# stevebottos/owl-vit-object-detection

Hardware: AMD Instinct MI355X
Metric: train images/sec, OWL-ViT-B/16 768x768 (higher is better)
Workload: dtype bf16; 1 GPU; owlvit-base-patch16 bf16, batch=32/GPU, 768x768, full train step (matcher+loss+backward+AdamW); global_batch=32, parallelism=dp1, encoder_streams=2, weights=init, optimizer_schedule=in-line, windows=1

## Files before the change

### owl-vit-object-detection_amd/csrc/gemm_common.h

```cpp
#pragma once
#include "common.h"

constexpr int NUM_CUS = 256;

enum {
    EPI_BIAS_BF16 = 0,
    EPI_QGELU_BF16 = 1,
    EPI_GELU_BF16 = 2,
    EPI_RESID_F32 = 3,
    EPI_F32 = 4,
    EPI_ATOMIC_F32 = 5,
    EPI_TRANS_BF16 = 6,
    EPI_PATCH_F32 = 7,
    EPI_DQGELU_BF16 = 8,
    EPI_DGELU_BF16 = 9,
    EPI_ACC_F32 = 10,
    EPI_SLAB_F32 = 11,
    EPI_PATCHM_F32 = 12,
};

struct GemmP {
    const bf16_t* A; int64_t lda; int64_t a_rows;
    const bf16_t* W; int64_t ldw; int64_t w_rows;
    const float* bias;
// ... 121 lines not shown
        *(float4*)((float*)p.out + orow * p.ldo + n) = make_float4(r4.x + v[0], r4.y + v[1], r4.z + v[2], r4.w + v[3]);
    } else if constexpr (EPI == EPI_F32) {
        *(float4*)((float*)p.out + orow * p.ldo + n) = make_float4(v[0], v[1], v[2], v[3]);
    } else if constexpr (EPI == EPI_SLAB_F32) {
        *(float4*)((float*)p.out + (int64_t)split * p.slab_stride + orow * p.ldo + n) = make_float4(v[0], v[1], v[2], v[3]);
    } else if constexpr (EPI == EPI_PATCH_F32 || EPI == EPI_PATCHM_F32) {
        const float4 p4 = *(const float4*)(posrow + n);
        *(float4*)((float*)p.out + orow * p.ldo + n) = make_float4(v[0] + p4.x, v[1] + p4.y, v[2] + p4.z, v[3] + p4.w);
    } else if constexpr (EPI == EPI_ATOMIC_F32) {
        float* o = (float*)p.out + orow * p.ldo + n;
#pragma unroll
        for (int e = 0; e < 4; e++) atomicAdd(o + e, v[e]);
    }
}

template <int EPI>
__device__ __forceinline__ void epi_pass(const GemmP& p, const f32x16& t0, const f32x16& t1, unsigned char* pieceA,
                                         unsigned char* pieceB, int64_t row_base, int64_t col_base, int lane, int split) {
    constexpr bool TRANS = (EPI == EPI_TRANS_BF16);
    const int hi = lane >> 5, r = lane & 31;
    unsigned char* wrow = (r < 16 ? pieceA : pieceB) + (r & 15) * 256;
#pragma unroll
    for (int qd = 0; qd < 4; qd++) {
        const int c0 = 2 * qd + hi, c1 = 8 + c0;
        *(float4*)(wrow + ((c0 ^ (r & 15)) << 4)) = make_float4(t0[qd * 4 + 0], t0[qd * 4 + 1], t0[qd * 4 + 2], t0[qd * 4 + 3]);
        *(float4*)(wrow + ((c1 ^ (r & 15)) << 4)) = make_float4(t1[qd * 4 + 0], t1[qd * 4 + 1], t1[qd * 4 + 2], t1[qd * 4 + 3]);
    }
    const int ch = lane & 15;
#pragma unroll
    for (int it = 0; it < 8; it++) {
        const int row = it * 4 + (lane >> 4);
        const unsigned char* rrow = (row < 16 ? pieceA : pieceB) + (row & 15) * 256;
        const f32x4 f = lds_read_f4(rrow + ((ch ^ (row & 15)) << 4));
        float v[4] = {f[0], f[1], f[2], f[3]};
        if constexpr (!TRANS) {
            const int64_t m = row_base + row, n = col_base + ch * 4;
            if (m >= p.M || n >= p.N) continue;
            int64_t orow = m;
            const float* posrow = nullptr;
            if constexpr (EPI == EPI_PATCH_F32 || EPI == EPI_PATCHM_F32) {
                const int64_t b = m / p.P, pp = m - b * p.P;
                orow = b * p.Tp + 1 + pp;
                posrow = p.pos + (1 + pp) * p.N;
            }
            epi_quad<EPI>(p, orow, posrow, n, v, split);
        } else {
            const int64_t n = row_base + row, m = col_base + ch * 4;
            if (n >= p.N || m >= p.M) continue;
            const float bv = p.bias ? p.bias[n] : 0.f;
            const int64_t b = m / p.Tp, t = m - b * p.Tp;
            uint2 o;
            o.x = pack_bf2(v[0] + bv, v[1] + bv);
            o.y = pack_bf2(v[2] + bv, v[3] + bv);
            *(uint2*)((bf16_t*)p.out + (b * p.N + n) * p.Tp + t) = o;
        }
    }
}

__device__ __forceinline__ void epi_bias_preload(const float* lds_bias, int hi, f32x4 (&bq)[2][4]) {
    const unsigned a = (unsigned)(uintptr_t)LPTR(lds_bias + 4 * hi);
    asm volatile("ds_read_b128 %0, %8\n\tds_read_b128 %1, %8 offset:32\n\tds_read_b128 %2, %8 offset:64\n\tds_read_b128 %3, %8 offset:96\n\t"
                 "ds_read_b128 %4, %8 offset:128\n\tds_read_b128 %5, %8 offset:160\n\tds_read_b128 %6, %8 offset:192\n\tds_read_b128 %7, %8 offset:224\n\t"
                 "s_waitcnt lgkmcnt(0)"
                 : "=&v"(bq[0][0]), "=&v"(bq[0][1]), "=&v"(bq[0][2]), "=&v"(bq[0][3]), "=&v"(bq[1][0]), "=&v"(bq[1][1]), "=&v"(bq[1][2]), "=&v"(bq[1][3])
                 : "v"(a) : "memory");
}

template <bool GUARD>
__device__ __forceinline__ void epi_aux_load(const GemmP& p, int64_t m_tile, int64_t n_tile, int lane, uint4 (&a)[2]) {
    const int hi = lane >> 5;
    const int64_t m = m_tile + (lane & 31);
#pragma unroll
    for (int c = 0; c < 2; c++) {
        const int64_t n = n_tile + 16 * c + 8 * hi;
        a[c] = make_uint4(0u, 0u, 0u, 0u);
        if (!GUARD || (m < p.M && n < p.N)) a[c] = *(const uint4*)((const bf16_t*)p.aux + m * p.ld_aux + n);
    }
}

template <int EPI, bool GUARD>
__device__ __forceinline__ void epi_tile_bf16(const GemmP& p, const f32x16& acc, int64_t m_tile, int64_t n_tile, int lane,
                                              uint4& chunk0, uint4& chunk1, const float* lds_bias, const uint4* aux_pre = nullptr,
                                              const f32x4* bias_pre = nullptr) {
    constexpr bool TRANS = (EPI == EPI_TRANS_BF16);
    const int hi = lane >> 5;
    unsigned w[8];
    unsigned aw[8] = {};
    if constexpr (TRANS) {
        const int64_t n = n_tile + (lane & 31);
        float bv = 0.f;
        if (p.bias) bv = lds_read_f1(lds_bias + (lane & 31));
#pragma unroll
        for (int qd = 0; qd < 4; qd++) {
            w[2 * qd] = pack_bf2(acc[qd * 4 + 0] + bv, acc[qd * 4 + 1] + bv);
            w[2 * qd + 1] = pack_bf2(acc[qd * 4 + 2] + bv, acc[qd * 4 + 3] + bv);
        }
    } else {
        const int64_t m = m_tile + (lane & 31);
        const bool m_ok = !GUARD || m < p.M;
        const bf16_t* aux_row = (const bf16_t*)p.aux + m * p.ld_aux + n_tile + 4 * hi;
        const float* bias_p = lds_bias + 4 * hi;
        if constexpr (EPI == EPI_DQGELU_BF16 || EPI == EPI_DGELU_BF16) {
            if (aux_pre) {
                unsigned ax[4] = {aux_pre[0].x, aux_pre[0].y, aux_pre[1].x, aux_pre[1].y}, ay[4] = {aux_pre[0].z, aux_pre[0].w, aux_pre[1].z, aux_pre[1].w};
#pragma unroll
                for (int k = 0; k < 4; k++) {
                    auto r = __builtin_amdgcn_permlane32_swap(ax[k], ay[k], false, false);
                    ax[k] = r[0]; ay[k] = r[1];
                }
                aw[0] = ax[0]; aw[1] = ax[1]; aw[2] = ay[0]; aw[3] = ay[1]; aw[4] = ax[2]; aw[5] = ax[3]; aw[6] = ay[2]; aw[7] = ay[3];
            }
        }
#pragma unroll
        for (int qd = 0; qd < 4; qd++) {
            float v[4];
            const bool n_ok = !GUARD || (n_tile + 8 * qd + 4 * hi) < p.N;
            const bool ok = m_ok && n_ok;
            const f32x2_t al = {p.alpha, p.alpha};
            f32x2_t b01 = {0.f, 0.f}, b23 = {0.f, 0.f};
            if (p.bias) {
                const f32x4 b4 = bias_pre ? bias_pre[qd] : lds_read_f4(bias_p + 8 * qd);
                b01 = (f32x2_t){b4[0], b4[1]}; b23 = (f32x2_t){b4[2], b4[3]};
            }
            const f32x2_t v01 = __builtin_elementwise_fma((f32x2_t){acc[qd * 4 + 0], acc[qd * 4 + 1]}, al, b01);
            const f32x2_t v23 = __builtin_elementwise_fma((f32x2_t){acc[qd * 4 + 2], acc[qd * 4 + 3]}, al, b23);
            v[0] = v01.x; v[1] = v01.y; v[2] = v23.x; v[3] = v23.y;
            if constexpr (EPI == EPI_QGELU_BF16 || EPI == EPI_GELU_BF16) {
                float sv[4] = {v[0], v[1], v[2], v[3]};
                if constexpr (EPI == EPI_QGELU_BF16) {
#pragma unroll
                    for (int e = 0; e < 4; e += 2) {
                        const f32x2_t u = {v[e], v[e + 1]};
                        const f32x2_t t = u * -2.4554669595930156f;
                        const f32x2_t d = (f32x2_t){__builtin_amdgcn_exp2f(t.x), __builtin_amdgcn_exp2f(t.y)} + 1.0f;
                        const f32x2_t r = {__builtin_amdgcn_rcpf(d.x), __builtin_amdgcn_rcpf(d.y)};
                        const f32x2_t o = u * r;
                        if (p.aux) { sv[e] = dqgelu_from_s(u.x, r.x); sv[e + 1] = dqgelu_from_s(u.y, r.y); }
                        v[e] = o.x; v[e + 1] = o.y;
                    }
                } else {
#pragma unroll
                    for (int e = 0; e < 4; e++) v[e] = gelu_f(v[e]);
                }
                if (p.aux) {
                    if constexpr (EPI == EPI_QGELU_BF16) {
                        aw[2 * qd] = pack_bf2(sv[0], sv[1]); aw[2 * qd + 1] = pack_bf2(sv[2], sv[3]);
                    } else {
                        uint2 a; a.x = pack_bf2(sv[0], sv[1]); a.y = pack_bf2(sv[2], sv[3]);
                        if (ok) *(uint2*)((bf16_t*)aux_row + 8 * qd) = a;
                    }
                }
            } else if constexpr (EPI == EPI_DQGELU_BF16 || EPI == EPI_DGELU_BF16) {
                uint2 a = make_uint2(0u, 0u);
                if (aux_pre) a = make_uint2(aw[2 * qd], aw[2 * qd + 1]);
                else if (ok) a = *(const uint2*)(aux_row + 8 * qd);
                const float u[4] = {bf2f(a.x & 0xffff), bf2f(a.x >> 16), bf2f(a.y & 0xffff), bf2f(a.y >> 16)};
#pragma unroll
                for (int e = 0; e < 4; e++) v[e] *= (EPI == EPI_DQGELU_BF16) ? u[e] : dgelu_f(u[e]);
            }
            w[2 * qd] = pack_bf2(v[0], v[1]);
            w[2 * qd + 1] = pack_bf2(v[2], v[3]);
        }
    }
    if constexpr (!TRANS && EPI == EPI_QGELU_BF16) {
        if (p.aux) {
            unsigned ax[4] = {aw[0], aw[1], aw[4], aw[5]}, ay[4] = {aw[2], aw[3], aw[6], aw[7]};
#pragma unroll
            for (int k = 0; k < 4; k++) {
                auto r = __builtin_amdgcn_permlane32_swap(ax[k], ay[k], false, false);
                ax[k] = r[0]; ay[k] = r[1];
            }
            typedef __attribute__((ext_vector_type(4))) unsigned u32x4_t;
            const int64_t m = m_tile + (lane & 31);
            bf16_t* arow = (bf16_t*)p.aux + m * p.ld_aux + n_tile + 8 * hi;
            const u32x4_t s0 = {ax[0], ax[1], ay[0], ay[1]}, s1 = {ax[2], ax[3], ay[2], ay[3]};
            if (!GUARD || (m < p.M && n_tile + 8 * hi < p.N)) *(u32x4_t*)arow = s0;
            if (!GUARD || (m < p.M && n_tile + 16 + 8 * hi < p.N)) *(u32x4_t*)(arow + 16) = s1;
        }
    }
    unsigned x[4] = {w[0], w[1], w[4], w[5]}, y[4] = {w[2], w[3], w[6], w[7]};
#pragma unroll
    for (int k = 0; k < 4; k++) {
        auto r = __builtin_amdgcn_permlane32_swap(x[k], y[k], false, false);
        x[k] = r[0]; y[k] = r[1];
    }
    chunk0 = make_uint4(x[0], x[1], y[0], y[1]);
    chunk1 = make_uint4(x[2], x[3], y[2], y[3]);
}


__device__ __forceinline__ void epi_lines_bias_preload(const float* lds_bias, int hi, f32x4 (&bq)[8]) {
    const unsigned a = (unsigned)(uintptr_t)LPTR(lds_bias + 32 * hi);
    asm volatile("ds_read_b128 %0, %8\n\tds_read_b128 %1, %8 offset:16\n\tds_read_b128 %2, %8 offset:32\n\tds_read_b128 %3, %8 offset:48\n\t"
                 "ds_read_b128 %4, %8 offset:64\n\tds_read_b128 %5, %8 offset:80\n\tds_read_b128 %6, %8 offset:96\n\tds_read_b128 %7, %8 offset:112\n\t"
                 "s_waitcnt lgkmcnt(0)"
                 : "=&v"(bq[0]), "=&v"(bq[1]), "=&v"(bq[2]), "=&v"(bq[3]), "=&v"(bq[4]), "=&v"(bq[5]), "=&v"(bq[6]), "=&v"(bq[7])
                 : "v"(a) : "memory");
}

__device__ __forceinline__ void quad_transpose16(unsigned (&d)[16], int lane) {
    const bool o1 = lane & 1, o2 = lane & 2;
#pragma unroll
    for (int c = 0; c < 4; c++) {
#pragma unroll
        for (int g = 0; g < 2; g++) {
            unsigned& x = d[8 * g + c]; unsigned& y = d[8 * g + 4 + c];
            const unsigned u = (unsigned)__builtin_amdgcn_mov_dpp((int)(o1 ? x : y), 0xB1, 0xF, 0xF, true);
            if (o1) x = u; else y = u;
        }
#pragma unroll
        for (int g = 0; g < 2; g++) {
            unsigned& x = d[4 * g + c]; unsigned& y = d[4 * g + 8 + c];
            const unsigned u = (unsigned)__builtin_amdgcn_mov_dpp((int)(o2 ? x : y), 0x4E, 0xF, 0xF, true);
            if (o2) x = u; else y = u;
        }
    }
}

template <bool GUARD>
__device__ __forceinline__ void epi_lines_aux_load(const GemmP& p, int64_t m_tile, int64_t n_wave, int lane, unsigned (&x)[16]) {
    typedef __attribute__((ext_vector_type(4))) unsigned u32x4_t;
    const int hi = lane >> 5;
    const bf16_t* base = (const bf16_t*)p.aux + m_tile * p.ld_aux + n_wave;
    const unsigned ld = (unsigned)p.ld_aux, col = 32u * hi + 8u * (lane & 3), r0 = (unsigned)(lane & 28);
#pragma unroll
    for (int t = 0; t < 4; t++) {
        u32x4_t v = {0u, 0u, 0u, 0u};
        if (!GUARD || (m_tile + r0 + t < p.M && n_wave + col < p.N)) v = *(const u32x4_t*)(base + ((r0 + t) * ld + col));
        x[4 * t] = v[0]; x[4 * t + 1] = v[1]; x[4 * t + 2] = v[2]; x[4 * t + 3] = v[3];
    }
}

template <int EPI, bool GUARD>
__device__ __forceinline__ void epi_lines_bf16(const GemmP& p, const f32x16& acc0, const f32x16& acc1, int64_t m_tile, int64_t n_wave, int lane,
                                               const float* lds_bias, const f32x4* bias_pre = nullptr,
                                               unsigned* aux_words = nullptr) {
    static_assert(EPI == EPI_BIAS_BF16 || EPI == EPI_QGELU_BF16 || EPI == EPI_GELU_BF16 || EPI == EPI_DQGELU_BF16,
                  "quad-contiguous epilogue: forward bf16 epilogues and the multiply-by-saved-derivative one");
    const int hi = lane >> 5;
    const int64_t m = m_tile + (lane & 31);
    const float* bias_p = lds_bias + 32 * hi;
    unsigned d_own[16], a[16];
    unsigned (&d)[16] = (EPI == EPI_DQGELU_BF16) ? *reinterpret_cast<unsigned (*)[16]>(aux_words) : d_own;
#pragma unroll
    for (int j = 0; j < 2; j++)
#pragma unroll
        for (int qd = 0; qd < 4; qd++) {
            const f32x16& acc = j ? acc1 : acc0;
            float v[4];
            const f32x2_t al = {p.alpha, p.alpha};
            f32x2_t b01 = {0.f, 0.f}, b23 = {0.f, 0.f};
            if (p.bias) {
                const f32x4 b4 = bias_pre ? bias_pre[4 * j + qd] : lds_read_f4(bias_p + 16 * j + 4 * qd);
                b01 = (f32x2_t){b4[0], b4[1]}; b23 = (f32x2_t){b4[2], b4[3]};
            }
            const f32x2_t v01 = __builtin_elementwise_fma((f32x2_t){acc[qd * 4 + 0], acc[qd * 4 + 1]}, al, b01);
            const f32x2_t v23 = __builtin_elementwise_fma((f32x2_t){acc[qd * 4 + 2], acc[qd * 4 + 3]}, al, b23);
            v[0] = v01.x; v[1] = v01.y; v[2] = v23.x; v[3] = v23.y;
            if constexpr (EPI == EPI_QGELU_BF16 || EPI == EPI_GELU_BF16) {
                float sv[4] = {v[0], v[1], v[2], v[3]};
                if constexpr (EPI == EPI_QGELU_BF16) {
#pragma unroll
                    for (int e = 0; e < 4; e += 2) {
                        const f32x2_t u = {v[e], v[e + 1]};
                        const f32x2_t t = u * -2.4554669595930156f;
                        const f32x2_t dd = (f32x2_t){__builtin_amdgcn_exp2f(t.x), __builtin_amdgcn_exp2f(t.y)} + 1.0f;
                        const f32x2_t r = {__builtin_amdgcn_rcpf(dd.x), __builtin_amdgcn_rcpf(dd.y)};
                        const f32x2_t o = u * r;
                        if (p.aux) { sv[e] = dqgelu_from_s(u.x, r.x); sv[e + 1] = dqgelu_from_s(u.y, r.y); }
                        v[e] = o.x; v[e + 1] = o.y;
                    }
                } else {
#pragma unroll
                    for (int e = 0; e < 4; e++) v[e] = gelu_f(v[e]);
                }
                if (p.aux) { a[8 * j + 2 * qd] = pack_bf2(sv[0], sv[1]); a[8 * j + 2 * qd + 1] = pack_bf2(sv[2], sv[3]); }
            } else if constexpr (EPI == EPI_DQGELU_BF16) {
                const unsigned a0 = aux_words[8 * j + 2 * qd], a1 = aux_words[8 * j + 2 * qd + 1];
                v[0] *= bf2f(a0 & 0xffff); v[1] *= bf2f(a0 >> 16); v[2] *= bf2f(a1 & 0xffff); v[3] *= bf2f(a1 >> 16);
            }
            d[8 * j + 2 * qd] = pack_bf2(v[0], v[1]);
            d[8 * j + 2 * qd + 1] = pack_bf2(v[2], v[3]);
        }
    typedef __attribute__((ext_vector_type(4))) unsigned u32x4_t;
    if constexpr (EPI == EPI_QGELU_BF16 || EPI == EPI_GELU_BF16) {
        if (p.aux) {
            bf16_t* aux_row = (bf16_t*)p.aux + m * p.ld_aux + n_wave + 32 * hi;
#pragma unroll
            for (int t = 0; t < 4; t++)
                if (!GUARD || (m < p.M && n_wave + 32 * hi + 8 * t < p.N))
                    *(u32x4_t*)(aux_row + 8 * t) = (u32x4_t){a[4 * t], a[4 * t + 1], a[4 * t + 2], a[4 * t + 3]};
        }
    }
    quad_transpose16(d, lane);
    const int64_t row0 = m_tile + (lane & 28), n = n_wave + 32 * hi + 8 * (lane & 3);
#pragma unroll
    for (int t = 0; t < 4; t++) {
        const int64_t row = row0 + t;
        if (GUARD && (row >= p.M || n >= p.N)) continue;
        *(u32x4_t*)((bf16_t*)p.out + row * p.ldo + n) = (u32x4_t){d[4 * t], d[4 * t + 1], d[4 * t + 2], d[4 * t + 3]};
    }
}

template <int EPI, bool GUARD>
__device__ __forceinline__ void epi_tile_f32(const GemmP& p, const f32x16& acc, int64_t m_tile, int64_t n_tile, int lane, const float* lds_bias,
                                             const f32x4* bias_pre = nullptr) {
    const int hi = lane >> 5;
    const int64_t m = m_tile + (lane & 31);
    const bool m_ok = !GUARD || m < p.M;
    float* orow = (float*)p.out + m * p.ldo + n_tile + 4 * hi;
    const float* bias_p = lds_bias + 4 * hi;
#pragma unroll
    for (int qd = 0; qd < 4; qd++) {
        float v[4];
#pragma unroll
        for (int e = 0; e < 4; e++) v[e] = acc[qd * 4 + e] * p.alpha;
        if (p.bias) {
            const f32x4 b4 = bias_pre ? bias_pre[qd] : lds_read_f4(bias_p + 8 * qd);
            v[0] += b4[0]; v[1] += b4[1]; v[2] += b4[2]; v[3] += b4[3];
        }
        const bool ok = m_ok && (!GUARD || (n_tile + 8 * qd + 4 * hi) < p.N);
        if (!ok) continue;
        if constexpr (EPI == EPI_ACC_F32) {
            const float4 r4 = *(const float4*)(orow + 8 * qd);
            *(float4*)(orow + 8 * qd) = make_float4(r4.x + v[0], r4.y + v[1], r4.z + v[2], r4.w + v[3]);
        } else {
            *(float4*)(orow + 8 * qd) = make_float4(v[0], v[1], v[2], v[3]);
        }
    }
}

template <bool GUARD>
__device__ __forceinline__ void epi_tile_patch(const GemmP& p, const f32x16& acc, int64_t m_tile, int64_t n_tile, int lane) {
    const int hi = lane >> 5;
    const int64_t m = m_tile + (lane & 31);
    const bool m_ok = !GUARD || m < p.M;
    const int64_t mm = m_ok ? m : 0;
    const int64_t b = mm / p.P, pp = mm - b * p.P;
    float* orow = (float*)p.out + (b * p.Tp + 1 + pp) * p.ldo + n_tile + 4 * hi;
    const float* prow = p.pos + (1 + pp) * p.N + n_tile + 4 * hi;
#pragma unroll
    for (int qd = 0; qd < 4; qd++) {
        if (!m_ok || (GUARD && (n_tile + 8 * qd + 4 * hi) >= p.N)) continue;
        const float4 p4 = *(const float4*)(prow + 8 * qd);
        *(float4*)(orow + 8 * qd) = make_float4(acc[qd * 4 + 0] * p.alpha + p4.x, acc[qd * 4 + 1] * p.alpha + p4.y,
                                                acc[qd * 4 + 2] * p.alpha + p4.z, acc[qd * 4 + 3] * p.alpha + p4.w);
    }
}

template <int EPI, bool GUARD>
__device__ __forceinline__ void epi_store_chunk(const GemmP& p, const uint4& ch, int64_t m_tile, int64_t n_tile, int c, int lane) {
    const int hi = lane >> 5;
    if constexpr (EPI == EPI_TRANS_BF16) {
        const int64_t n = n_tile + (lane & 31), m = m_tile + 16 * c + 8 * hi;
        if (GUARD && (n >= p.N || m >= p.M)) return;
        const int64_t b = m / p.Tp, t = m - b * p.Tp;
        *(uint4*)((bf16_t*)p.out + (b * p.N + n) * p.Tp + t) = ch;
    } else {
        int64_t m = m_tile + (lane & 31), n = n_tile + 16 * c + 8 * hi;
        if (GUARD && (m >= p.M || n >= p.N)) return;
#ifdef OWL_TUNING
        if (p.dbg & 2) { m = (int64_t)(blockIdx.x & 255) * 256 + (m & 255); n &= 255; }
#endif
        typedef __attribute__((ext_vector_type(4))) unsigned u32x4_t;
        u32x4_t* dst = (u32x4_t*)((bf16_t*)p.out + m * p.ldo + n);
        const u32x4_t val = {ch.x, ch.y, ch.z, ch.w};
#ifdef OWL_TUNING
        if (p.dbg & 4) { __builtin_nontemporal_store(val, dst); return; }
#endif
        *dst = val;
    }
}
```

### owl-vit-object-detection_amd/csrc/gemm_pp2.hip

```cpp
#include "gemm_common.h"
#include <type_traits>

static constexpr int QBM = 256, QBN = 256, QBK = 64;
static constexpr int Q_A_BYTES = QBM * QBK * 2, Q_B_BYTES = QBN * QBK * 2, Q_STAGE = Q_A_BYTES + Q_B_BYTES;
static constexpr int Q_BIAS_OFF = 2 * Q_STAGE, Q_LDS = 2 * Q_STAGE + 2 * 1024;

template <int N> __device__ __forceinline__ void q_wait() { asm volatile("s_waitcnt vmcnt(%0) lgkmcnt(0)" ::"n"(N) : "memory"); }
__device__ __forceinline__ void q_wait_lgkm() { asm volatile("s_waitcnt lgkmcnt(0)" ::: "memory"); }
__device__ __forceinline__ void q_bar() {
    __builtin_amdgcn_sched_barrier(0);
    __builtin_amdgcn_s_barrier();
    asm volatile("" ::: "memory");
    __builtin_amdgcn_sched_barrier(0);
}

template <int EPI, bool TRACE = false, bool LINES = false>
__global__ __launch_bounds__(512) void gemm_pp2_kernel(GemmP p) {
    extern __shared__ __attribute__((aligned(16))) unsigned char lds[];
    const int lane = threadIdx.x & 63;
    const int w = __builtin_amdgcn_readfirstlane(threadIdx.x >> 6);
    const int hi = lane >> 5;
    const int grp = w >> 2, wc = w & 3;
    const int nk = (int)(p.K / QBK);
    const int nitems = p.tiles_m * p.tiles_n;
    const int bw = p.nsplit;
    auto decode = [&](int it, int& tm, int& tn) {
        const int per_block = p.tiles_m * bw;
        const int cb = it / per_block, rem = it - cb * per_block;
        tm = rem / bw; tn = cb * bw + (rem - tm * bw);
    };
    int item, item_end, item_step;
    if (p.persistent) {
        const int xcd = blockIdx.x & 7, idx = blockIdx.x >> 3, chunk = (nitems + 7) >> 3;
        item = xcd * chunk + idx; item_end = min(nitems, (xcd + 1) * chunk); item_step = gridDim.x >> 3;
    } else {
        item = xcd_remap(blockIdx.x, nitems); item_end = item + 1; item_step = 1;
    }
    if (item >= item_end) return;
    if (p.stagger > 0 && ((blockIdx.x >> 3) & 1))
        for (int i = 0; i < p.stagger; i++) __builtin_amdgcn_s_sleep(127);
#ifdef OWL_TUNING
    const bool abl_nodma = (p.dbg >> 16) & 1, abl_noread = (p.dbg >> 17) & 1, abl_noepi = (p.dbg >> 18) & 1;
    bool abl_prologue = true;
#else
    constexpr bool abl_nodma = false, abl_noread = false, abl_noepi = false, abl_prologue = true;
#endif

    int a_item = item, a_k = 0, a_buf = 0;
    int b_item = item, b_k = 0, b_buf = 0, b_parity = 0;
    unsigned a_voff[2][2], w_voff[2][2], b_voff = 0;
    const bf16_t* a_base = nullptr;
    const bf16_t* w_base = nullptr;
    const float* b_base = nullptr;
    const bool has_bias = p.bias != nullptr;
    constexpr bool GATHER = (EPI == EPI_PATCH_F32);
    const bool np2 = GATHER && p.ps != (int64_t(1) << p.ps_log2);
    int a_j[2] = {0, 0};
    auto stage_A = [&]() {
        if (a_k == 0) {
            int tm, tn_unused; decode(a_item, tm, tn_unused);
            const int64_t m0 = (int64_t)tm * QBM;
            a_base = GATHER ? p.A : p.A + m0 * p.lda;
#pragma unroll
            for (int h = 0; h < 2; h++)
#pragma unroll
                for (int q = 0; q < 2; q++) {
                    const int r = h * 128 + (w * 2 + q) * 8 + (lane >> 3);
                    const int c = (lane & 7) ^ ((r >> 1) & 7);
                    int64_t am = m0 + r; if (am >= p.a_rows) am = p.a_rows - 1;
                    if constexpr (GATHER) {
                        const unsigned P32 = (unsigned)p.P, G32 = (unsigned)p.G, S32 = (unsigned)p.S, ps32 = (unsigned)p.ps;
                        const unsigned b = (unsigned)am / P32, pp = (unsigned)am - b * P32;
                        const unsigned py = pp / G32, px = pp - py * G32;
                        unsigned ky = (unsigned)(c * 8) >> p.ps_log2, kx = (unsigned)(c * 8) & ((1u << p.ps_log2) - 1u);
                        if (np2) { a_j[q] = (int)ky; ky = 0; kx = min(kx, ps32 - 8u); }
                        a_voff[h][q] = ((((b * 3u) * S32 + py * ps32 + ky) * S32) + px * ps32 + kx) * 2u;
                    } else {
                        a_voff[h][q] = (unsigned)(((am - m0) * p.lda + c * 8) * 2);
                    }
                }
        }
        unsigned char* base = lds + a_buf * Q_STAGE;
        int64_t koff = (int64_t)a_k * QBK;
        unsigned roff[2] = {0u, 0u};
        if constexpr (GATHER) {
            if (np2) {
                koff = 0;
#pragma unroll
                for (int q = 0; q < 2; q++) {
                    unsigned R = (unsigned)(a_k * (QBK >> p.ps_log2) + a_j[q]);
                    R = min(R, 3u * (unsigned)p.ps - 1u);
                    const unsigned ch = (R * (unsigned)p.ps_magic) >> 16, ky = R - ch * (unsigned)p.ps;
                    roff[q] = ((ch * (unsigned)p.S + ky) * (unsigned)p.S) * 2u;
                }
            } else {
                const int k = a_k * QBK;
                const int ch = k >> (2 * p.ps_log2), ky = (k & ((1 << (2 * p.ps_log2)) - 1)) >> p.ps_log2;
                koff = ((int64_t)ch * p.S + ky) * p.S;
            }
        }
        const unsigned char* g = (const unsigned char*)(a_base + koff);
        if (!abl_nodma || abl_prologue) {
#pragma unroll
        for (int h = 0; h < 2; h++)
#pragma unroll
            for (int q = 0; q < 2; q++)
                __builtin_amdgcn_global_load_lds(GPTR(g + (a_voff[h][q] + roff[q])), LPTR(base + (h * 128 + (w * 2 + q) * 8) * 128), 16, 0, 0);
        }
        a_buf ^= 1;
        if (++a_k == nk) { a_k = 0; a_item += item_step; }
    };
    auto stage_B = [&]() -> int {
        const bool first = b_k == 0;
        if (first) {
            int tm, tn; decode(b_item, tm, tn);
            const int64_t n0 = (int64_t)tn * QBN;
            w_base = p.W + n0 * p.ldw;
#pragma unroll
            for (int h = 0; h < 2; h++)
#pragma unroll
                for (int q = 0; q < 2; q++) {
                    const int r = h * 128 + (w * 2 + q) * 8 + (lane >> 3);
                    const int c = (lane & 7) ^ ((r >> 1) & 7);
                    const int rs = LINES ? ((r & ~63) | (((r >> 2) & 1) << 5) | (((r >> 5) & 1) << 4) | (((r >> 3) & 3) << 2) | (r & 3)) : r;
                    int64_t wn = n0 + rs; if (wn >= p.w_rows) wn = p.w_rows - 1;
                    w_voff[h][q] = (unsigned)(((wn - n0) * p.ldw + c * 8) * 2);
                }
            if (has_bias) {
                int64_t n = n0 + lane * 4; if (n + 4 > p.N) n = p.N - 4;
                b_base = p.bias + n0;
                b_voff = (unsigned)((n - n0) * 4);
            }
        }
        unsigned char* base = lds + b_buf * Q_STAGE + Q_A_BYTES;
        const unsigned char* g = (const unsigned char*)(w_base + (int64_t)b_k * QBK);
        int n_ops = 0;
        if (!abl_nodma || abl_prologue) {
#pragma unroll
        for (int h = 0; h < 2; h++)
#pragma unroll
            for (int q = 0; q < 2; q++)
                __builtin_amdgcn_global_load_lds(GPTR(g + w_voff[h][q]), LPTR(base + (h * 128 + (w * 2 + q) * 8) * 128), 16, 0, 0);
        n_ops = 4;
        if (first && has_bias) {
            __builtin_amdgcn_global_load_lds(GPTR((const unsigned char*)b_base + b_voff), LPTR(lds + Q_BIAS_OFF + b_parity * 1024), 16, 0, 0);
            n_ops = 5;
        }
        }
        b_buf ^= 1;
        if (++b_k == nk) { b_k = 0; b_item += item_step; b_parity ^= 1; }
        return n_ops;
    };

    const int a_frag_off = frag_off<false>(grp * 128, lane), b_frag_off = Q_A_BYTES + frag_off<true>(wc * 64, lane);

    stage_B(); stage_A(); stage_B();
    q_wait<4>();
    q_bar();
#ifdef OWL_TUNING
    abl_prologue = false;
#endif

    int cur = 0, tile_parity = 0;
    const bool tr_wg = TRACE && blockIdx.x == 0;
    bool tr_first = false;
    int tr_tile = 0;
    if (TRACE && (p.dbg >> 8) == 0) tr_first = true;
    unsigned long long tr_ts[12] = {};
    bool a_early = false;
    int pending_stores = 0;
    constexpr bool STAGGERED_EPI = ((EPI == EPI_BIAS_BF16 && !LINES) || EPI == EPI_F32 || EPI == EPI_ACC_F32 || EPI == EPI_PATCH_F32 || EPI == EPI_PATCHM_F32);
    if (STAGGERED_EPI && grp == 1) q_bar();
    unsigned long long wg_t0 = 0;
    unsigned long long wg_r0 = 0;
    if constexpr (TRACE) asm volatile("s_memtime %0\n\ts_memrealtime %1\n\ts_waitcnt lgkmcnt(0)" : "=s"(wg_t0), "=s"(wg_r0) :: "memory");
    unsigned long long tile_ts[5] = {};
    auto tile_stamp = [&](int i) {
        if constexpr (TRACE) { if (tr_wg && tr_first) asm volatile("s_memtime %0\n\ts_waitcnt lgkmcnt(0)" : "=s"(tile_ts[i]) :: "memory"); }
    };
    while (true) {
        tile_stamp(0);
        AccBlock blk[4][2];
#pragma unroll
        for (int i = 0; i < 4; i++)
#pragma unroll
            for (int j = 0; j < 2; j++) acc_block_zero(blk[i][j]);
        int tm, tn; decode(item, tm, tn);
        const int64_t cm0 = (int64_t)tm * QBM, cn0 = (int64_t)tn * QBN;
        if (!STAGGERED_EPI && grp == 1) q_bar();
        tile_stamp(1);
        for (int kt = 0; kt < nk; kt++) {
            const unsigned char* tb = lds + cur * Q_STAGE;
            auto stamp = [&](int idx) {
                if constexpr (TRACE) {
                    if (tr_wg && tr_first && kt == ((p.dbg >> 4) & 15)) {
                        if (idx == 1 || idx == 6) return;
                        if (idx == 0 || idx == 2 || idx == 7 || idx >= 10) asm volatile("s_memtime %0\n\ts_waitcnt lgkmcnt(0)" : "=s"(tr_ts[idx]));
                        else asm volatile("s_memtime %0" : "=s"(tr_ts[idx]));
                    }
                }
            };
            bf16x8 fa[2][4], fb[2][4];
            auto ld_a = [&](int ih) {
#pragma unroll
                for (int t = 0; t < 2; t++)
#pragma unroll
                    for (int x = 0; x < 4; x++) fa[t][x] = frag_read(tb + (2 * ih + t) * 4096, a_frag_off, x >> 1, x & 1);
            };
            auto mma = [&](int ih) {
                __builtin_amdgcn_s_setprio(1);
#pragma unroll
                for (int s = 0; s < 2; s++)
#pragma unroll
                    for (int t = 0; t < 2; t++)
#pragma unroll
                        for (int j = 0; j < 2; j++) mma_block_step(blk[2 * ih + t][j], fb[j], fa[t], s);
                __builtin_amdgcn_s_setprio(0);
            };
            stamp(0);
            if (!abl_noread || kt == 0) {
#pragma unroll
            for (int j = 0; j < 2; j++)
#pragma unroll
                for (int x = 0; x < 4; x++) fb[j][x] = frag_read(tb + j * 4096, b_frag_off, x >> 1, x & 1);
            ld_a(0);
            }
            if (a_early) a_early = false;
            else if (a_item < item_end) stage_A();
            stamp(1);
            q_wait_lgkm();
            stamp(2);
            q_bar();
            stamp(3);
            mma(0);
            stamp(4);
            q_bar();
            stamp(5);
            if (!abl_noread || kt == 0) ld_a(1);
            int n_new = 0;
            if (b_item < item_end) n_new = stage_B();
            stamp(6);
            switch (n_new + pending_stores) {
                case 4: q_wait<4>(); break;
                case 5: q_wait<5>(); break;
                case 20: q_wait<20>(); break;
                case 21: q_wait<21>(); break;
                case 36: q_wait<36>(); break;
                case 37: q_wait<37>(); break;
                default: q_wait<0>(); break;
            }
            pending_stores = 0;
            stamp(7);
            q_bar();
            stamp(8);
            mma(1);
            stamp(9);
            q_bar();
            stamp(10);
            if constexpr (TRACE) {
                if (tr_wg && tr_first && kt == ((p.dbg >> 4) & 15) && lane == 0) {
#pragma unroll
                    for (int i = 0; i < 11; i++) ((unsigned long long*)(lds + Q_LDS))[w * 16 + i] = tr_ts[i];
                }
            }
            cur ^= 1;
        }
        tile_stamp(2);
        f32x16 acc[4][2];
#pragma unroll
        for (int i = 0; i < 4; i++)
#pragma unroll
            for (int j = 0; j < 2; j++) acc[i][j] = acc_block_32x32(blk[i][j]);
        if (!STAGGERED_EPI && grp == 0) q_bar();
        const bool inner = (cm0 + QBM <= p.M) && (cn0 + QBN <= p.N);
        constexpr bool PLAIN_EPI = (EPI == EPI_BIAS_BF16 || EPI == EPI_QGELU_BF16 || EPI == EPI_GELU_BF16);
        constexpr bool AUX_COUNTED = (EPI == EPI_QGELU_BF16);
        if (PLAIN_EPI && inner && (AUX_COUNTED || !p.aux) && a_item < item_end) { stage_A(); a_early = true; pending_stores = (AUX_COUNTED && p.aux) ? 32 : 16; }
        const float* lbias = (const float*)(lds + Q_BIAS_OFF + tile_parity * 1024) + wc * 64;
        auto estamp = [&](int idx) {
            if constexpr (TRACE) { if (tr_wg && tr_first && ((p.dbg >> 4) & 15) == 15) asm volatile("s_memtime %0\n\ts_waitcnt lgkmcnt(0)" : "=s"(tr_ts[idx]) :: "memory"); }
        };
        auto run = [&](auto guard_tag) {
            constexpr bool G = decltype(guard_tag)::value;
            estamp(0);
            constexpr bool AUX_IN = (EPI == EPI_DQGELU_BF16);
            uint4 auxr[AUX_IN ? 2 : 1][2][2];
            if constexpr (AUX_IN && !LINES) {
#pragma unroll
                for (int i = 0; i < 2; i++)
#pragma unroll
                    for (int j = 0; j < 2; j++) epi_aux_load<G>(p, cm0 + grp * 128 + i * 32, cn0 + wc * 64 + j * 32, lane, auxr[i][j]);
            }
            constexpr bool BIAS_PRE = (EPI == EPI_BIAS_BF16 || EPI == EPI_QGELU_BF16 || EPI == EPI_F32 || EPI == EPI_ACC_F32);
            f32x4 bq[2][4];
            if constexpr (BIAS_PRE && !LINES) { if (has_bias) epi_bias_preload(lbias, hi, bq); }
            if constexpr (LINES && AUX_IN) {
                unsigned ax[2][16];
                epi_lines_aux_load<G>(p, cm0 + grp * 128, cn0 + wc * 64, lane, ax[0]);
                epi_lines_aux_load<G>(p, cm0 + grp * 128 + 32, cn0 + wc * 64, lane, ax[1]);
                estamp(1);
#pragma unroll
                for (int i = 0; i < 4; i++) {
                    quad_transpose16(ax[i & 1], lane);
                    epi_lines_bf16<EPI, G>(p, acc[i][0], acc[i][1], cm0 + grp * 128 + i * 32, cn0 + wc * 64, lane, lbias, nullptr, ax[i & 1]);
                    if (i + 2 < 4) epi_lines_aux_load<G>(p, cm0 + grp * 128 + (i + 2) * 32, cn0 + wc * 64, lane, ax[i & 1]);
                    estamp(2 + i);
                }
            } else if constexpr (LINES) {
                f32x4 bl[8];
                if (has_bias) epi_lines_bias_preload(lbias, hi, bl);
                estamp(1);
#pragma unroll
                for (int i = 0; i < 4; i++) {
                    epi_lines_bf16<EPI, G>(p, acc[i][0], acc[i][1], cm0 + grp * 128 + i * 32, cn0 + wc * 64, lane, lbias, bl);
                    estamp(2 + i);
                }
            } else {
            estamp(1);
#pragma unroll
            for (int i = 0; i < 4; i++) {
#pragma unroll
                for (int j = 0; j < 2; j++) {
                    const int64_t mt = cm0 + grp * 128 + i * 32, nt = cn0 + wc * 64 + j * 32;
                    if constexpr (EPI == EPI_F32 || EPI == EPI_ACC_F32) {
                        epi_tile_f32<EPI, G>(p, acc[i][j], mt, nt, lane, lbias + j * 32, BIAS_PRE ? bq[j] : nullptr);
                    } else if constexpr (EPI == EPI_PATCH_F32 || EPI == EPI_PATCHM_F32) {
                        epi_tile_patch<G>(p, acc[i][j], mt, nt, lane);
                    } else {
                        uint4 c0, c1;
                        epi_tile_bf16<EPI, G>(p, acc[i][j], mt, nt, lane, c0, c1, lbias + j * 32, AUX_IN ? auxr[AUX_IN ? (i & 1) : 0][j] : nullptr, BIAS_PRE ? bq[j] : nullptr);
                        if constexpr (AUX_IN) { if (i + 2 < 4) epi_aux_load<G>(p, mt + 64, nt, lane, auxr[i & 1][j]); }
                        epi_store_chunk<EPI, G>(p, c0, mt, nt, 0, lane);
                        epi_store_chunk<EPI, G>(p, c1, mt, nt, 1, lane);
                    }
                }
                estamp(2 + i);
            }
            }
        };
        if (!abl_noepi) {
            if (inner) run(std::false_type{}); else run(std::true_type{});
        } else {
            pending_stores = 0;
#pragma unroll
            for (int i = 0; i < 4; i++)
#pragma unroll
                for (int j = 0; j < 2; j++) asm volatile("" :: "v"(acc[i][j]));
        }
        tile_stamp(4);
        if (STAGGERED_EPI) q_bar();
        tile_stamp(3);
        if constexpr (TRACE) {
            if (tr_wg && tr_first) {
                if (lane == 0 && ((p.dbg >> 4) & 15) == 15) {
#pragma unroll
                    for (int i = 0; i < 11; i++) ((unsigned long long*)(lds + Q_LDS))[w * 16 + i] = tr_ts[i];
                }
                if (lane == 0) {
#pragma unroll
                    for (int i = 0; i < 5; i++) ((unsigned long long*)(lds + Q_LDS))[w * 16 + 11 + i] = tile_ts[i];
                }
                __syncthreads();
                if (threadIdx.x < 128) ((unsigned long long*)p.aux)[threadIdx.x] = ((unsigned long long*)(lds + Q_LDS))[threadIdx.x];
                tr_first = false;
            }
            if (tr_wg && ++tr_tile == (p.dbg >> 8) && !tr_first) tr_first = true;
        }
        item += item_step;
        if (item >= item_end) break;
        tile_parity ^= 1;
    }
    if (STAGGERED_EPI && grp == 0) q_bar();
    if constexpr (TRACE) {
        unsigned long long wg_t1, wg_r1;
        asm volatile("s_waitcnt vmcnt(0)\n\ts_memtime %0\n\ts_memrealtime %1\n\ts_waitcnt lgkmcnt(0)" : "=s"(wg_t1), "=s"(wg_r1) :: "memory");
        if (threadIdx.x == 0) {
            ((unsigned long long*)p.aux)[128 + blockIdx.x] = wg_t1 - wg_t0; ((unsigned long long*)p.aux)[128 + 256 + blockIdx.x] = wg_r0;
            ((unsigned long long*)p.aux)[128 + 512 + blockIdx.x] = wg_r1;
        }
    }
}

#ifdef OWL_TUNING
static int g_pp2_nostore = 0;
OWL_API int owl_gemm_pp2_nostore(int on) { g_pp2_nostore = on; return 0; }
static int g_pp2_slots = 256;
OWL_API int owl_gemm_pp2_slots(int n) { g_pp2_slots = n; return 0; }
static int g_pp2_bw[2] = {0, 0};
OWL_API int owl_gemm_pp2_block_width(int epi, int bw) { if (epi < 0 || epi > 1) return -1; g_pp2_bw[epi] = bw; return 0; }
static int g_pp2_abl = 0;
OWL_API int owl_gemm_pp2_ablate(int a) { g_pp2_abl = a; return 0; }
static int g_pp2_lines = 1;
OWL_API int owl_gemm_pp2_lines(int on) { g_pp2_lines = on; return 0; }
static int g_pp2_stagger = 0;
OWL_API int owl_gemm_pp2_stagger(int n) { g_pp2_stagger = n; return 0; }
#else
static constexpr int g_pp2_slots = 256;
#endif

template <int EPI>
static int launch_pp2(hipStream_t s, GemmP p) {
    static unsigned long long attr_done = 0;
    OWL_ONCE_PER_DEVICE(attr_done, {
        (void)hipFuncSetAttribute((const void*)gemm_pp2_kernel<EPI>, hipFuncAttributeMaxDynamicSharedMemorySize, Q_LDS);
    });
    p.tiles_m = (int)((p.M + QBM - 1) / QBM); p.tiles_n = (int)((p.N + QBN - 1) / QBN);
    p.dbg = 0;
    p.stagger = 0;
#ifdef OWL_TUNING
    p.dbg = g_pp2_abl << 16;
    p.stagger = g_pp2_stagger;
#endif
    p.nsplit = p.tiles_n;
    if (EPI == EPI_BIAS_BF16 || EPI == EPI_QGELU_BF16)
        for (int d = (EPI == EPI_QGELU_BF16 && p.tiles_m > 160) ? 6 : 4; d >= 1; d--)
            if (p.tiles_n % d == 0) { p.nsplit = d; break; }
#ifdef OWL_TUNING
    if constexpr (EPI == EPI_BIAS_BF16 || EPI == EPI_QGELU_BF16) {
        const int want = g_pp2_bw[EPI == EPI_QGELU_BF16 ? 1 : 0];
        if (want > 0)
            for (int d = want; d >= 1; d--)
                if (p.tiles_n % d == 0) { p.nsplit = d; break; }
    }
#endif
    const int nitems = p.tiles_m * p.tiles_n;
#ifdef OWL_TUNING
    if (g_pp2_nostore) p.M = 0;
#endif
    p.persistent = nitems > g_pp2_slots ? 1 : 0;
#ifdef OWL_TUNING
    constexpr bool LINES_OK = (EPI == EPI_BIAS_BF16 || EPI == EPI_QGELU_BF16 || EPI == EPI_DQGELU_BF16);
    const bool lines_on = EPI == EPI_BIAS_BF16 ? g_pp2_lines >= 1 : (EPI == EPI_DQGELU_BF16 ? g_pp2_lines >= 3 : g_pp2_lines >= 2);
#else
    constexpr bool LINES_OK = (EPI == EPI_BIAS_BF16);
    const bool lines_on = true;
#endif
    if constexpr (LINES_OK) {
        if (lines_on && p.N % 8 == 0) {
            static unsigned long long attr_done_l = 0;
            OWL_ONCE_PER_DEVICE(attr_done_l, {
                (void)hipFuncSetAttribute((const void*)gemm_pp2_kernel<EPI, false, true>, hipFuncAttributeMaxDynamicSharedMemorySize, Q_LDS);
            });
            hipLaunchKernelGGL((gemm_pp2_kernel<EPI, false, true>), dim3(p.persistent ? g_pp2_slots : nitems), dim3(512), Q_LDS, s, p);
            OWL_LAUNCH_CHECK();
            return 0;
        }
    }
    hipLaunchKernelGGL((gemm_pp2_kernel<EPI>), dim3(p.persistent ? g_pp2_slots : nitems), dim3(512), Q_LDS, s, p);
    OWL_LAUNCH_CHECK();
    return 0;
}

#ifdef OWL_TUNING
static void* g_pp2_trace = nullptr;
static int g_pp2_trace_tile = 0, g_pp2_trace_kt = 4;
OWL_API int owl_gemm_pp2_trace(void* buf) { g_pp2_trace = buf; return 0; }
OWL_API int owl_gemm_pp2_trace_tile(int n) { g_pp2_trace_tile = n; return 0; }
OWL_API int owl_gemm_pp2_trace_ktile(int n) { g_pp2_trace_kt = n; return 0; }
#endif

int owl_gemm_pp2_launch(hipStream_t s, int epi, const GemmP& p) {
#ifdef OWL_TUNING
    if (g_pp2_trace && epi == EPI_BIAS_BF16) {
        GemmP q = p;
        q.aux = nullptr;
        (void)hipFuncSetAttribute((const void*)gemm_pp2_kernel<EPI_BIAS_BF16, true>, hipFuncAttributeMaxDynamicSharedMemorySize, Q_LDS + 2048);
        q.tiles_m = (int)((q.M + QBM - 1) / QBM); q.tiles_n = (int)((q.N + QBN - 1) / QBN); q.dbg = (g_pp2_trace_tile << 8) | ((g_pp2_trace_kt & 15) << 4); q.nsplit = q.tiles_n;
        for (int d = 4; d >= 1; d--) if (q.tiles_n % d == 0) { q.nsplit = d; break; }
        const int nitems = q.tiles_m * q.tiles_n;
        q.persistent = nitems > 256 ? 1 : 0;
        GemmP qq = q; qq.aux = g_pp2_trace;
        if (g_pp2_lines) {
            (void)hipFuncSetAttribute((const void*)gemm_pp2_kernel<EPI_BIAS_BF16, true, true>, hipFuncAttributeMaxDynamicSharedMemorySize, Q_LDS + 2048);
            hipLaunchKernelGGL((gemm_pp2_kernel<EPI_BIAS_BF16, true, true>), dim3(q.persistent ? 256 : nitems), dim3(512), Q_LDS + 2048, s, qq);
            return 0;
        }
        hipLaunchKernelGGL((gemm_pp2_kernel<EPI_BIAS_BF16, true>), dim3(q.persistent ? 256 : nitems), dim3(512), Q_LDS + 2048, s, qq);
        return 0;
    }
#endif
    switch (epi) {
        case EPI_BIAS_BF16: return launch_pp2<EPI_BIAS_BF16>(s, p);
        case EPI_QGELU_BF16: return launch_pp2<EPI_QGELU_BF16>(s, p);
        case EPI_DQGELU_BF16: return launch_pp2<EPI_DQGELU_BF16>(s, p);
        case EPI_GELU_BF16: return launch_pp2<EPI_GELU_BF16>(s, p);
        case EPI_DGELU_BF16: return launch_pp2<EPI_DGELU_BF16>(s, p);
        case EPI_F32: return launch_pp2<EPI_F32>(s, p);
        case EPI_ACC_F32: return launch_pp2<EPI_ACC_F32>(s, p);
        case EPI_PATCH_F32: return launch_pp2<EPI_PATCH_F32>(s, p);
        case EPI_PATCHM_F32: return launch_pp2<EPI_PATCHM_F32>(s, p);
        default: owl_set_error("owl_gemm_pp2_launch: epilogue %d is not one of pp2_takes (planner and launcher disagree)", epi); return -1;
    }
}
```

Before: 1243 images/sec.

## Add quad-contiguous line-store epilogue for f32 GEMM outputs with prefetched reads

Extends the LINES epilogue path, previously used only for bf16 bias output, to the f32, accumulate-f32 and patch-embedding f32 epilogues. Accumulators are quad-transposed so each lane writes contiguous 16-byte row pieces. Residual and positional-embedding reads are issued early with inline-asm loads and explicit vmcnt waits, and the next tile's A staging is started before the epilogue. This aims to make global stores and reads more coalesced and to overlap them with compute, at the cost of alignment preconditions, more register pressure, and fp-contract-off rounding changes.

```diff
diff --git a/owl-vit-object-detection_amd/csrc/gemm_common.h b/owl-vit-object-detection_amd/csrc/gemm_common.h
--- a/owl-vit-object-detection_amd/csrc/gemm_common.h
+++ b/owl-vit-object-detection_amd/csrc/gemm_common.h
@@ -447,50 +447,155 @@
     }
 }
 
-template <int EPI, bool GUARD>
+template <int EPI, bool GUARD, bool LCOLS = false>
 __device__ __forceinline__ void epi_tile_f32(const GemmP& p, const f32x16& acc, int64_t m_tile, int64_t n_tile, int lane, const float* lds_bias,
                                              const f32x4* bias_pre = nullptr) {
+#pragma clang fp contract(off)
     const int hi = lane >> 5;
+    constexpr int CS = LCOLS ? 4 : 8;
+    const int c0 = LCOLS ? 32 * hi : 4 * hi;
     const int64_t m = m_tile + (lane & 31);
     const bool m_ok = !GUARD || m < p.M;
-    float* orow = (float*)p.out + m * p.ldo + n_tile + 4 * hi;
-    const float* bias_p = lds_bias + 4 * hi;
+    float* orow = (float*)p.out + m * p.ldo + n_tile + c0;
+    const float* bias_p = lds_bias + c0;
 #pragma unroll
     for (int qd = 0; qd < 4; qd++) {
         float v[4];
 #pragma unroll
         for (int e = 0; e < 4; e++) v[e] = acc[qd * 4 + e] * p.alpha;
         if (p.bias) {
-            const f32x4 b4 = bias_pre ? bias_pre[qd] : lds_read_f4(bias_p + 8 * qd);
-            v[0] += b4[0]; v[1] += b4[1]; v[2] += b4[2]; v[3] += b4[3];
-        }
-        const bool ok = m_ok && (!GUARD || (n_tile + 8 * qd + 4 * hi) < p.N);
+            const f32x4 b4 = bias_pre ? bias_pre[qd] : lds_read_f4(bias_p + CS * qd);
+            v[0] = v[0] + b4[0]; v[1] = v[1] + b4[1]; v[2] = v[2] + b4[2]; v[3] = v[3] + b4[3];
+        }
+        const bool ok = m_ok && (!GUARD || (n_tile + CS * qd + c0) < p.N);
         if (!ok) continue;
         if constexpr (EPI == EPI_ACC_F32) {
-            const float4 r4 = *(const float4*)(orow + 8 * qd);
-            *(float4*)(orow + 8 * qd) = make_float4(r4.x + v[0], r4.y + v[1], r4.z + v[2], r4.w + v[3]);
+            const float4 r4 = *(const float4*)(orow + CS * qd);
+            *(float4*)(orow + CS * qd) = make_float4(r4.x + v[0], r4.y + v[1], r4.z + v[2], r4.w + v[3]);
         } else {
-            *(float4*)(orow + 8 * qd) = make_float4(v[0], v[1], v[2], v[3]);
-        }
-    }
-}
-
-template <bool GUARD>
+            *(float4*)(orow + CS * qd) = make_float4(v[0], v[1], v[2], v[3]);
+        }
+    }
+}
+
+template <bool GUARD, bool LCOLS = false>
 __device__ __forceinline__ void epi_tile_patch(const GemmP& p, const f32x16& acc, int64_t m_tile, int64_t n_tile, int lane) {
     const int hi = lane >> 5;
+    constexpr int CS = LCOLS ? 4 : 8;
+    const int c0 = LCOLS ? 32 * hi : 4 * hi;
     const int64_t m = m_tile + (lane & 31);
     const bool m_ok = !GUARD || m < p.M;
     const int64_t mm = m_ok ? m : 0;
     const int64_t b = mm / p.P, pp = mm - b * p.P;
-    float* orow = (float*)p.out + (b * p.Tp + 1 + pp) * p.ldo + n_tile + 4 * hi;
-    const float* prow = p.pos + (1 + pp) * p.N + n_tile + 4 * hi;
+    float* orow = (float*)p.out + (b * p.Tp + 1 + pp) * p.ldo + n_tile + c0;
+    const float* prow = p.pos + (1 + pp) * p.N + n_tile + c0;
 #pragma unroll
     for (int qd = 0; qd < 4; qd++) {
-        if (!m_ok || (GUARD && (n_tile + 8 * qd + 4 * hi) >= p.N)) continue;
-        const float4 p4 = *(const float4*)(prow + 8 * qd);
-        *(float4*)(orow + 8 * qd) = make_float4(acc[qd * 4 + 0] * p.alpha + p4.x, acc[qd * 4 + 1] * p.alpha + p4.y,
-                                                acc[qd * 4 + 2] * p.alpha + p4.z, acc[qd * 4 + 3] * p.alpha + p4.w);
-    }
+        if (!m_ok || (GUARD && (n_tile + CS * qd + c0) >= p.N)) continue;
+        const float4 p4 = *(const float4*)(prow + CS * qd);
+        *(float4*)(orow + CS * qd) = make_float4(acc[qd * 4 + 0] * p.alpha + p4.x, acc[qd * 4 + 1] * p.alpha + p4.y,
+                                                 acc[qd * 4 + 2] * p.alpha + p4.z, acc[qd * 4 + 3] * p.alpha + p4.w);
+    }
+}
+
+template <int EPI>
+struct LinesF32Rows {
+    float* base;
+    unsigned off[4];
+    unsigned poff[4];
+
+    __device__ __forceinline__ void init(const GemmP& p, int64_t m_tile, int64_t n_wave, int lane) {
+        const unsigned r0 = (unsigned)(lane & 28), col = 32u * (unsigned)(lane >> 5) + 4u * (unsigned)(lane & 3), ld = (unsigned)p.ldo;
+        if constexpr (EPI == EPI_PATCH_F32) {
+            const unsigned P32 = (unsigned)p.P, Tp32 = (unsigned)p.Tp, N32 = (unsigned)p.N;
+            const unsigned mt = (unsigned)m_tile, bt = mt / P32, orow_t = bt * Tp32 + 1u + (mt - bt * P32);
+            base = (float*)p.out + (int64_t)orow_t * p.ldo + n_wave;
+            unsigned b = (mt + r0) / P32, pp = (mt + r0) - b * P32;
+#pragma unroll
+            for (int t = 0; t < 4; t++) {
+                off[t] = (b * Tp32 + 1u + pp - orow_t) * ld + col;
+                poff[t] = (1u + pp) * N32 + col;
+                if (++pp == P32) { pp = 0u; b++; }
+            }
+        } else {
+            base = (float*)p.out + m_tile * p.ldo + n_wave;
+#pragma unroll
+            for (int t = 0; t < 4; t++) { off[t] = (r0 + t) * ld + col; poff[t] = 0u; }
+        }
+    }
+};
+
+template <int EPI>
+__device__ __forceinline__ void epi_lines_f32_load(const GemmP& p, const LinesF32Rows<EPI>& rw, int64_t n_wave, int j, f32x4 (&x)[4]) {
+    static_assert(EPI == EPI_ACC_F32 || EPI == EPI_PATCH_F32, "only these read");
+    const float* pbase = p.pos + n_wave;
+#pragma unroll
+    for (int t = 0; t < 4; t++) {
+        const float* src = (EPI == EPI_ACC_F32) ? rw.base + (rw.off[t] + 16u * j) : pbase + (rw.poff[t] + 16u * j);
+        asm volatile("global_load_dwordx4 %0, %1, off" : "=v"(x[t]) : "v"(src) : "memory");
+    }
+}
+
+template <int N>
+__device__ __forceinline__ void epi_lines_f32_wait(f32x4 (&x)[4]) {
+    asm volatile("s_waitcnt vmcnt(%4)" : "+v"(x[0]), "+v"(x[1]), "+v"(x[2]), "+v"(x[3]) : "n"(N));
+}
+
+template <int EPI, int WAIT>
+__device__ __forceinline__ void epi_lines_f32_tile(const GemmP& p, const f32x16& acc, int j, int lane, const float* lds_bias, const f32x4* bias_pre,
+                                                   f32x4 (&x)[4], f32x4 (&o)[4]) {
+#pragma clang fp contract(off)
+    const float* bias_p = lds_bias + 32 * (lane >> 5);
+    unsigned d[16];
+#pragma unroll
+    for (int qd = 0; qd < 4; qd++) {
+        float v[4];
+#pragma unroll
+        for (int e = 0; e < 4; e++) v[e] = acc[qd * 4 + e];
+        if constexpr (EPI != EPI_PATCH_F32) {
+#pragma unroll
+            for (int e = 0; e < 4; e++) v[e] = v[e] * p.alpha;
+            if (p.bias) {
+                const f32x4 b4 = bias_pre ? bias_pre[4 * j + qd] : lds_read_f4(bias_p + 16 * j + 4 * qd);
+                v[0] = v[0] + b4[0]; v[1] = v[1] + b4[1]; v[2] = v[2] + b4[2]; v[3] = v[3] + b4[3];
+            }
+        }
+#pragma unroll
+        for (int e = 0; e < 4; e++) d[qd * 4 + e] = __float_as_uint(v[e]);
+    }
+    quad_transpose16(d, lane);
+    if constexpr (EPI != EPI_F32) epi_lines_f32_wait<WAIT>(x);
+#pragma unroll
+    for (int t = 0; t < 4; t++)
+#pragma unroll
+        for (int e = 0; e < 4; e++) {
+            const float v = __uint_as_float(d[4 * t + e]);
+            if constexpr (EPI == EPI_ACC_F32) o[t][e] = x[t][e] + v;
+            else if constexpr (EPI == EPI_PATCH_F32) o[t][e] = fmaf(v, p.alpha, x[t][e]);
+            else o[t][e] = v;
+        }
+}
+
+template <int EPI>
+__device__ __forceinline__ void epi_lines_f32_store(const LinesF32Rows<EPI>& rw, int j, const f32x4 (&o)[4]) {
+#pragma unroll
+    for (int t = 0; t < 4; t++) *(f32x4*)(rw.base + (rw.off[t] + 16u * j)) = o[t];
+}
+
+template <int EPI, bool FIRST, bool LAST>
+__device__ __forceinline__ void epi_lines_f32(const GemmP& p, const f32x16& acc0, const f32x16& acc1, const LinesF32Rows<EPI>& rw,
+                                              const LinesF32Rows<EPI>& next, int64_t n_wave, int lane, const float* lds_bias,
+                                              const f32x4* bias_pre, f32x4 (&x)[2][4]) {
+    static_assert(EPI == EPI_F32 || EPI == EPI_ACC_F32 || EPI == EPI_PATCH_F32, "quad-contiguous f32 epilogue");
+    constexpr bool READS = (EPI == EPI_ACC_F32 || EPI == EPI_PATCH_F32);
+    f32x4 o[4];
+    epi_lines_f32_tile<EPI, FIRST ? 0 : 8>(p, acc0, 0, lane, lds_bias, bias_pre, x[0], o);
+    if constexpr (READS && FIRST) epi_lines_f32_load<EPI>(p, rw, n_wave, 1, x[1]);
+    epi_lines_f32_store<EPI>(rw, 0, o);
+    if constexpr (READS && !LAST) epi_lines_f32_load<EPI>(p, next, n_wave, 0, x[0]);
+    epi_lines_f32_tile<EPI, LAST ? 4 : 8>(p, acc1, 1, lane, lds_bias, bias_pre, x[1], o);
+    epi_lines_f32_store<EPI>(rw, 1, o);
+    if constexpr (READS && !LAST) epi_lines_f32_load<EPI>(p, next, n_wave, 1, x[1]);
 }
 
 template <int EPI, bool GUARD>
diff --git a/owl-vit-object-detection_amd/csrc/gemm_pp2.hip b/owl-vit-object-detection_amd/csrc/gemm_pp2.hip
--- a/owl-vit-object-detection_amd/csrc/gemm_pp2.hip
+++ b/owl-vit-object-detection_amd/csrc/gemm_pp2.hip
@@ -169,6 +169,7 @@
     unsigned long long tr_ts[12] = {};
     bool a_early = false;
     int pending_stores = 0;
+    constexpr bool F32_LINES = LINES && (EPI == EPI_F32 || EPI == EPI_ACC_F32 || EPI == EPI_PATCH_F32);
     constexpr bool STAGGERED_EPI = ((EPI == EPI_BIAS_BF16 && !LINES) || EPI == EPI_F32 || EPI == EPI_ACC_F32 || EPI == EPI_PATCH_F32 || EPI == EPI_PATCHM_F32);
     if (STAGGERED_EPI && grp == 1) q_bar();
     unsigned long long wg_t0 = 0;
@@ -276,6 +277,7 @@
         constexpr bool PLAIN_EPI = (EPI == EPI_BIAS_BF16 || EPI == EPI_QGELU_BF16 || EPI == EPI_GELU_BF16);
         constexpr bool AUX_COUNTED = (EPI == EPI_QGELU_BF16);
         if (PLAIN_EPI && inner && (AUX_COUNTED || !p.aux) && a_item < item_end) { stage_A(); a_early = true; pending_stores = (AUX_COUNTED && p.aux) ? 32 : 16; }
+        if (F32_LINES && inner && a_item < item_end) { stage_A(); a_early = true; pending_stores = (EPI == EPI_F32) ? 32 : 16; }
         const float* lbias = (const float*)(lds + Q_BIAS_OFF + tile_parity * 1024) + wc * 64;
         auto estamp = [&](int idx) {
             if constexpr (TRACE) { if (tr_wg && tr_first && ((p.dbg >> 4) & 15) == 15) asm volatile("s_memtime %0\n\ts_waitcnt lgkmcnt(0)" : "=s"(tr_ts[idx]) :: "memory"); }
@@ -305,6 +307,43 @@
                     epi_lines_bf16<EPI, G>(p, acc[i][0], acc[i][1], cm0 + grp * 128 + i * 32, cn0 + wc * 64, lane, lbias, nullptr, ax[i & 1]);
                     if (i + 2 < 4) epi_lines_aux_load<G>(p, cm0 + grp * 128 + (i + 2) * 32, cn0 + wc * 64, lane, ax[i & 1]);
                     estamp(2 + i);
+                }
+            } else if constexpr (F32_LINES) {
+                const int64_t mt0 = cm0 + grp * 128, nw = cn0 + wc * 64;
+                int lane = threadIdx.x & 63;
+                asm volatile("" : "+v"(lane));
+                if constexpr (G) {
+                    estamp(1);
+#pragma unroll
+                    for (int i = 0; i < 4; i++) {
+#pragma unroll
+                        for (int j = 0; j < 2; j++) {
+                            if constexpr (EPI == EPI_PATCH_F32) epi_tile_patch<true, true>(p, acc[i][j], mt0 + i * 32, nw + 16 * j, lane);
+                            else epi_tile_f32<EPI, true, true>(p, acc[i][j], mt0 + i * 32, nw + 16 * j, lane, lbias + 16 * j);
+                        }
+                        estamp(2 + i);
+                    }
+                } else {
+                    constexpr bool READS = (EPI != EPI_F32);
+                    f32x4 bl[EPI == EPI_F32 ? 8 : 1];
+                    if constexpr (EPI == EPI_F32) { if (has_bias) epi_lines_bias_preload(lbias, hi, bl); }
+                    LinesF32Rows<EPI> rw[2];
+                    f32x4 x[2][4];
+                    rw[0].init(p, mt0, nw, lane);
+                    if constexpr (READS) epi_lines_f32_load<EPI>(p, rw[0], nw, 0, x[0]);
+                    estamp(1);
+                    const f32x4* blp = EPI == EPI_F32 ? bl : nullptr;
+                    rw[1].init(p, mt0 + 32, nw, lane);
+                    epi_lines_f32<EPI, true, false>(p, acc[0][0], acc[0][1], rw[0], rw[1], nw, lane, lbias, blp, x);
+                    estamp(2);
+                    rw[0].init(p, mt0 + 64, nw, lane);
+                    epi_lines_f32<EPI, false, false>(p, acc[1][0], acc[1][1], rw[1], rw[0], nw, lane, lbias, blp, x);
+                    estamp(3);
+                    rw[1].init(p, mt0 + 96, nw, lane);
+                    epi_lines_f32<EPI, false, false>(p, acc[2][0], acc[2][1], rw[0], rw[1], nw, lane, lbias, blp, x);
+                    estamp(4);
+                    epi_lines_f32<EPI, false, true>(p, acc[3][0], acc[3][1], rw[1], rw[1], nw, lane, lbias, blp, x);
+                    estamp(5);
                 }
             } else if constexpr (LINES) {
                 f32x4 bl[8];
@@ -428,15 +467,18 @@
     if (g_pp2_nostore) p.M = 0;
 #endif
     p.persistent = nitems > g_pp2_slots ? 1 : 0;
-#ifdef OWL_TUNING
-    constexpr bool LINES_OK = (EPI == EPI_BIAS_BF16 || EPI == EPI_QGELU_BF16 || EPI == EPI_DQGELU_BF16);
-    const bool lines_on = EPI == EPI_BIAS_BF16 ? g_pp2_lines >= 1 : (EPI == EPI_DQGELU_BF16 ? g_pp2_lines >= 3 : g_pp2_lines >= 2);
+    constexpr bool LINES_F32 = (EPI == EPI_F32 || EPI == EPI_ACC_F32 || EPI == EPI_PATCH_F32);
+#ifdef OWL_TUNING
+    constexpr bool LINES_OK = (EPI == EPI_BIAS_BF16 || EPI == EPI_QGELU_BF16 || EPI == EPI_DQGELU_BF16 || LINES_F32);
+    const bool lines_on = (EPI == EPI_BIAS_BF16 || LINES_F32) ? g_pp2_lines >= 1 : (EPI == EPI_DQGELU_BF16 ? g_pp2_lines >= 3 : g_pp2_lines >= 2);
 #else
-    constexpr bool LINES_OK = (EPI == EPI_BIAS_BF16);
+    constexpr bool LINES_OK = (EPI == EPI_BIAS_BF16 || LINES_F32);
     const bool lines_on = true;
 #endif
     if constexpr (LINES_OK) {
-        if (lines_on && p.N % 8 == 0) {
+        const bool pieces_fit = LINES_F32 ? (p.N % 4 == 0 && p.ldo % 4 == 0 && (uintptr_t)p.out % 16 == 0 && (EPI != EPI_PATCH_F32 || (uintptr_t)p.pos % 16 == 0))
+                                          : p.N % 8 == 0;
+        if (lines_on && pieces_fit) {
             static unsigned long long attr_done_l = 0;
             OWL_ONCE_PER_DEVICE(attr_done_l, {
                 (void)hipFuncSetAttribute((const void*)gemm_pp2_kernel<EPI, false, true>, hipFuncAttributeMaxDynamicSharedMemorySize, Q_LDS);
```

Result: no change. 1247 images/sec, median of 6 (+0.3%).
